# AutonomousVehicleLaboratory/vision_semantic_segmentation

Hardware: AMD Instinct MI355X
Metric: fused frames/sec/GPU (1920x1080 + 120k pts) + max|dlog-odds| vs ref (higher is better)
Workload: dtype f16 hi+lo split, MX-FP4 correction passes, fp32 accumulate

## Files before the change

vision_semantic_segmentation_amd/csrc/seg_gconv_mfma.hip:

```cpp
#include <cstring>

#include "seg_types.h"

namespace avl {
namespace {

constexpr int TW = 32;
constexpr int CC = 64;

template <typename HT>
struct GconvArgs {
    const HT* in;
    const HT* in_lo;
    const HT* w;
    const float* bias;
    HT* out;
    HT* out_lo;
    char* oq[2];
    char* os[2];
    long long o_srows;
    int H, W, in_ld, OH, OW, out_ld, C;
    int stride, dil;
    int th;
    int tiles_x, tiles_y, cchunks;
    int comb;
    int nsp, nslots;
    int walk;
    int tile_bytes;
    int tw_magic;
    const char* w4;
    const char* w4s;
    const char* xq[2];
    const char* xs[2];
    long long x_srows;
    int dephase;
};

template <typename HT, int WS, int NJ, bool XS = false>
__global__ void __launch_bounds__(512) k_gconv_mfma(GconvArgs<HT> p) {
    static_assert(!XS || WS == 1, "a split input goes with split weights");
    typedef typename Half16<HT>::v8 v8;
    extern __shared__ __attribute__((aligned(16))) char lds[];
    const int tid = threadIdx.x, lane = tid & 63;
    const int wave = __builtin_amdgcn_readfirstlane(tid >> 6);
    {
        const long long ipix = (long long)p.H * p.W, opix = (long long)p.OH * p.OW;
        p.in = image_base(p.in, ipix, p.in_ld);
        p.in_lo = image_base(p.in_lo, ipix, p.in_ld);
        p.out = image_base(p.out, opix, p.out_ld);
        p.out_lo = image_base(p.out_lo, opix, p.out_ld);
#pragma unroll
        for (int pl = 0; pl < 2; ++pl) {
            p.oq[pl] = image_base(p.oq[pl], opix, p.C / 2);
            p.os[pl] = image_base(p.os[pl], opix, 8);
            p.xq[pl] = image_base(p.xq[pl], ipix, p.C / 2);
            p.xs[pl] = image_base(p.xs[pl], ipix, 8);
        }
    }
    int bid = blockIdx.x;
    {
        const int nwg = gridDim.x, xcd = bid & 7, local = bid >> 3, q = nwg >> 3, r = nwg & 7;
        bid = (xcd < r ? xcd * (q + 1) : r * (q + 1) + (xcd - r) * q) + local;
    }
    const int cchunk = bid % p.cchunks, slot = bid / p.cchunks;
    const int s = p.stride;
    const int d = p.comb ? 1 : p.dil;
    const int step = p.comb ? p.dil : 1;
    const int in_th = (p.th - 1) * s + 2 * d + 1, in_tw = (TW - 1) * s + 2 * d + 1;
    const int c0 = cchunk * CC;
    const int npix = in_th * in_tw;
    const int ngroups = (npix + 7) >> 3;
    const unsigned lds0 = lds_addr(lds);
    const int n64 = (npix + 63) >> 6;
    const int QBASE = ngroups * 1024, QT = n64 * 1024, SBASE = QBASE + 4 * QT, ST = n64 * 256;
    const bool has_lo = WS == 2 && p.xq[1] != nullptr;
    const int LOBASE = ngroups * 1024;

    const char* const xq0 = p.xq[0];
    const char* const xs0 = p.xs[0];
    const long long xq_delta = has_lo ? p.xq[1] - p.xq[0] : 0, xs_delta = has_lo ? p.xs[1] - p.xs[0] : 0;
    auto stage = [&](int sp, int buf) -> unsigned {
        int tx, ty, cmb;
        if (p.walk) { ty = sp % p.tiles_y; const int r1 = sp / p.tiles_y; tx = r1 % p.tiles_x; cmb = r1 / p.tiles_x; }
        else { tx = sp % p.tiles_x; const int r1 = sp / p.tiles_x; ty = r1 % p.tiles_y; cmb = r1 / p.tiles_y; }
        const int ry = p.comb ? cmb / p.dil : 0, rx = p.comb ? cmb % p.dil : 0;
        const int iy0 = ry + (ty * p.th * s - d) * step, ix0 = rx + (tx * TW * s - d) * step;
        const int prow = lane >> 3, cphys = lane & 7;
        unsigned oob = 0;
        int it = 0;
        for (int gi = wave; gi < ngroups; gi += 8, ++it) {
            const int pix = gi * 8 + prow;
            const int ly = (pix * p.tw_magic) >> 16, lx = pix - ly * in_tw;
            const int iy = iy0 + ly * step, ix = ix0 + lx * step;
            const unsigned outside = (unsigned)(pix >= npix) | (unsigned)((unsigned)iy >= (unsigned)p.H) | (unsigned)((unsigned)ix >= (unsigned)p.W);
            const int cy = min(max(iy, 0), p.H - 1), cx = min(max(ix, 0), p.W - 1);
            const unsigned voff = ((unsigned)(cy * p.W + cx) * (unsigned)p.in_ld + ((cphys ^ (pix & 7)) << 3)) * (unsigned)sizeof(HT);
            glds16_saddr(p.in + c0, voff, lds0 + buf * p.tile_bytes + gi * 1024);
            if constexpr (XS) glds16_saddr(p.in_lo + c0, voff, lds0 + buf * p.tile_bytes + LOBASE + gi * 1024);
            oob |= outside << it;
        }
        if constexpr (WS == 2) {
            const int pwbits = has_lo ? 2 : 1;
            it = 16;
            for (int item = wave; item < (n64 << pwbits); item += 8, ++it) {
                const int pw = item & ((1 << pwbits) - 1), gq = item >> pwbits, w = pw & 1, pl = pw >> 1;
                const int pix = gq * 64 + lane;
                const int ly = (pix * p.tw_magic) >> 16, lx = pix - ly * in_tw;
                const int iy = iy0 + ly * step, ix = ix0 + lx * step;
                const unsigned outside = (unsigned)(pix >= npix) | (unsigned)((unsigned)iy >= (unsigned)p.H) | (unsigned)((unsigned)ix >= (unsigned)p.W);
                const int cy = min(max(iy, 0), p.H - 1), cx = min(max(ix, 0), p.W - 1);
                glds16_saddr(xq0 + pl * xq_delta + c0 / 2 + w * 16, (unsigned)(cy * p.W + cx) * (unsigned)(p.C / 2),
                             lds0 + buf * p.tile_bytes + QBASE + (pl * 2 + w) * QT + gq * 1024);
                oob |= outside << it;
            }
            for (int item = wave; item < (n64 << (pwbits - 1)); item += 8) {
                const int pl = item & ((1 << (pwbits - 1)) - 1), gq = item >> (pwbits - 1);
                const int pix = gq * 64 + lane;
                const int ly = (pix * p.tw_magic) >> 16, lx = pix - ly * in_tw;
                const int cy = min(max(iy0 + ly * step, 0), p.H - 1), cx = min(max(ix0 + lx * step, 0), p.W - 1);
                glds4_saddr(xs0 + pl * xs_delta + ((long long)(c0 >> 8) * p.x_srows) * 8 + ((c0 >> 5) & 4), (unsigned)(cy * p.W + cx) * 8u,
                            lds0 + buf * p.tile_bytes + SBASE + pl * ST + gq * 256);
            }
        }
        return oob;
    };
    const int per = (p.nsp + p.nslots - 1) / p.nslots;
    const int sp_step = p.walk ? 1 : p.nslots, sp_end = p.walk ? min(p.nsp, (slot + 1) * per) : p.nsp;
    int sp = p.walk ? slot * per : slot, buf = 0;
    unsigned oob = sp < sp_end ? stage(sp, 0) : 0u;

    const int win = wave & 1;
    const int part = wave >> 1;
    const int fr = lane & 15, kq = lane >> 4;
    constexpr int NT = WS == 1 ? 18 : 9;
    v8 wf[2][NT];
    {
        const HT* wp = p.w + (long long)(cchunk * 2 + win) * (2 * NT * 16 * 32);
#pragma unroll
        for (int nj = 0; nj < 2; ++nj)
#pragma unroll
            for (int t = 0; t < NT; ++t)
                wf[nj][t] = *reinterpret_cast<const v8*>(wp + ((nj * NT + t) * 16 + fr) * 32 + kq * 8);
    }
    int4 w4[WS == 2 ? 2 : 1][2][3];
    unsigned w4sc[3] = {0u, 0u, 0u};
    if constexpr (WS == 2) {
        const long long widx = cchunk * 2 + win;
        const char* w4p = p.w4 + widx * (2 * 2 * 3 * 64 * 16) + lane * 16;
#pragma unroll
        for (int nj = 0; nj < 2; ++nj)
#pragma unroll
            for (int pr = 0; pr < 2; ++pr)
#pragma unroll
                for (int g = 0; g < 3; ++g) w4[nj][pr][g] = *reinterpret_cast<const int4*>(w4p + ((nj * 2 + pr) * 3 + g) * (64 * 16));
        const unsigned* sp = reinterpret_cast<const unsigned*>(p.w4s + widx * (64 * 12) + lane * 12);
        w4sc[0] = sp[0]; w4sc[1] = sp[1]; w4sc[2] = sp[2];
    }
    const int ssel = 8 * (((c0 >> 5) & 3) + win);
    const int cbase = c0 + win * 32 + kq * 8;
    const int chunk_in = win * 4 + kq;
    f32x4 bias0, bias1;
    {
        const float4 b0 = *reinterpret_cast<const float4*>(p.bias + cbase);
        const float4 b1 = *reinterpret_cast<const float4*>(p.bias + cbase + 4);
        bias0 = f32x4{b0.x, b0.y, b0.z, b0.w};
        bias1 = f32x4{b1.x, b1.y, b1.z, b1.w};
    }

    asm volatile("s_waitcnt vmcnt(0)" ::: "memory");
    auto zero_oob = [&](unsigned mask, int b) {
        if (mask) {
            int it = 0;
            for (int gi = wave; gi < ngroups; gi += 8, ++it)
                if ((mask >> it) & 1u) {
                    *reinterpret_cast<uint4*>(lds + b * p.tile_bytes + gi * 1024 + lane * 16) = make_uint4(0u, 0u, 0u, 0u);
                    if constexpr (XS) *reinterpret_cast<uint4*>(lds + b * p.tile_bytes + LOBASE + gi * 1024 + lane * 16) = make_uint4(0u, 0u, 0u, 0u);
                }
            if constexpr (WS == 2) {
                const int pwbits = has_lo ? 2 : 1;
                it = 16;
                for (int item = wave; item < (n64 << pwbits); item += 8, ++it)
                    if ((mask >> it) & 1u) {
                        const int pw = item & ((1 << pwbits) - 1), gq = item >> pwbits;
                        *reinterpret_cast<uint4*>(lds + b * p.tile_bytes + QBASE + pw * QT + gq * 1024 + lane * 16) = make_uint4(0u, 0u, 0u, 0u);
                    }
            }
        }
    };
    zero_oob(oob, 0);
    __syncthreads();

    constexpr bool HOIST = NJ <= 2 && WS != 2;
    int toff[HOIST ? NJ : 1][9];
    if constexpr (HOIST) {
#pragma unroll
        for (int j = 0; j < NJ; ++j) {
            const int st = part + 4 * j;
            const int sy = st >> 1, sx = (st & 1) * 16 + fr;
#pragma unroll
            for (int t = 0; t < 9; ++t) {
                const int pix = (sy * s + (t / 3) * d) * in_tw + sx * s + (t % 3) * d;
                toff[j][t] = pix * 128 + ((chunk_in ^ (pix & 7)) << 4);
            }
        }
    }
    const unsigned o_ld = (unsigned)p.out_ld, q_ld = (unsigned)(p.C / 2);
    const unsigned sc_lane = (unsigned)(cbase >> 8) * (unsigned)p.o_srows * 8u + (unsigned)((cbase >> 5) & 7);

    for (; sp < sp_end; sp += sp_step, buf ^= 1) {
        const bool late_stage = NJ >= 2 && wave >= 4 && p.dephase;
        oob = 0u;
        if (!late_stage && sp + sp_step < sp_end) oob = stage(sp + sp_step, buf ^ 1);
        const char* tile = lds + buf * p.tile_bytes;
        f32x4 acc[NJ][2];
#pragma unroll
        for (int j = 0; j < NJ; ++j) {
            if (NJ >= 2 && j == NJ / 2 && late_stage && sp + sp_step < sp_end) oob = stage(sp + sp_step, buf ^ 1);
            v8 a[9];
            if constexpr (HOIST) {
#pragma unroll
                for (int t = 0; t < 9; ++t) a[t] = *reinterpret_cast<const v8*>(tile + toff[j][t]);
            } else {
                const int st = part + 4 * j;
                int frv = fr;
                asm volatile("" : "+v"(frv));
                const int sy = st >> 1, sx = (st & 1) * 16 + frv;
#pragma unroll
                for (int t = 0; t < 9; ++t) {
                    const int pix = (sy * s + (t / 3) * d) * in_tw + sx * s + (t % 3) * d;
                    a[t] = *reinterpret_cast<const v8*>(tile + pix * 128 + ((chunk_in ^ (pix & 7)) << 4));
                }
            }
            f32x4 acc0 = bias0, acc1 = bias1;
            if constexpr (WS == 2) {
                typedef int v8i __attribute__((ext_vector_type(8)));
                const int st2 = part + 4 * j;
                const int sy2 = st2 >> 1, sx2 = (st2 & 1) * 16 + fr;
                int4 bq[2][3];
                int bs[2][3];
#pragma unroll
                for (int g = 0; g < 3; ++g) {
                    const int t = min(4 * g + kq, 8);
                    const int pix = (sy2 * s + (t / 3) * d) * in_tw + sx2 * s + (t % 3) * d;
#pragma unroll
                    for (int pl = 0; pl < 2; ++pl) {
                        if (pl == 1 && !has_lo) { bq[pl][g] = make_int4(0, 0, 0, 0); bs[pl][g] = 127; continue; }
                        bq[pl][g] = *reinterpret_cast<const int4*>(tile + QBASE + (pl * 2 + win) * QT + pix * 16);
                        bs[pl][g] = (int)((*reinterpret_cast<const unsigned*>(tile + SBASE + pl * ST + pix * 4) >> ssel) & 0xffu);
                    }
                }
#pragma unroll
                for (int t = 0; t < 9; ++t) {
                    acc0 = Half16<HT>::mfma(wf[0][t], a[t], acc0);
                    acc1 = Half16<HT>::mfma(wf[1][t], a[t], acc1);
                }
#define AVL_GMX(NJ_, PR, G, ACC)                                                                                                \
    {                                                                                                                          \
        const v8i wa = {w4[NJ_][PR][G].x, w4[NJ_][PR][G].y, w4[NJ_][PR][G].z, w4[NJ_][PR][G].w, 0, 0, 0, 0};                    \
        const v8i xa = {bq[PR][G].x, bq[PR][G].y, bq[PR][G].z, bq[PR][G].w, 0, 0, 0, 0};                                        \
        ACC = __builtin_amdgcn_mfma_scale_f32_16x16x128_f8f6f4(wa, xa, ACC, 4, 4, ((NJ_) * 6 + (PR) * 3 + (G)) & 3,              \
                                                               (int)w4sc[((NJ_) * 6 + (PR) * 3 + (G)) >> 2], 0, bs[PR][G]);     \
    }
                AVL_GMX(0, 0, 0, acc0) AVL_GMX(0, 0, 1, acc0) AVL_GMX(0, 0, 2, acc0)
                AVL_GMX(1, 0, 0, acc1) AVL_GMX(1, 0, 1, acc1) AVL_GMX(1, 0, 2, acc1)
                if (has_lo) {
                    AVL_GMX(0, 1, 0, acc0) AVL_GMX(0, 1, 1, acc0) AVL_GMX(0, 1, 2, acc0)
                    AVL_GMX(1, 1, 0, acc1) AVL_GMX(1, 1, 1, acc1) AVL_GMX(1, 1, 2, acc1)
                }
#undef AVL_GMX
            } else {
#pragma unroll
                for (int t = 0; t < 9; ++t) {
                    acc0 = Half16<HT>::mfma(wf[0][t], a[t], acc0);
                    acc1 = Half16<HT>::mfma(wf[1][t], a[t], acc1);
                    if constexpr (WS == 1) {
                        acc0 = Half16<HT>::mfma(wf[0][9 + t], a[t], acc0);
                        acc1 = Half16<HT>::mfma(wf[1][9 + t], a[t], acc1);
                    }
                }
                if constexpr (XS) {
                    if constexpr (HOIST) {
#pragma unroll
                        for (int t = 0; t < 9; ++t) a[t] = *reinterpret_cast<const v8*>(tile + LOBASE + toff[j][t]);
                    } else {
                        const int st = part + 4 * j;
                        int frv = fr;
                        asm volatile("" : "+v"(frv));
                        const int sy = st >> 1, sx = (st & 1) * 16 + frv;
#pragma unroll
                        for (int t = 0; t < 9; ++t) {
                            const int pix = (sy * s + (t / 3) * d) * in_tw + sx * s + (t % 3) * d;
                            a[t] = *reinterpret_cast<const v8*>(tile + LOBASE + pix * 128 + ((chunk_in ^ (pix & 7)) << 4));
                        }
                    }
#pragma unroll
                    for (int t = 0; t < 9; ++t) {
                        acc0 = Half16<HT>::mfma(wf[0][t], a[t], acc0);
                        acc1 = Half16<HT>::mfma(wf[1][t], a[t], acc1);
                    }
                }
            }
            acc[j][0] = acc0; acc[j][1] = acc1;
            __builtin_amdgcn_sched_barrier(0);
        }
        asm volatile("s_waitcnt vmcnt(0)" ::: "memory");
        zero_oob(oob, buf ^ 1);

        int tx, ty, cmb;
        if (p.walk) { ty = sp % p.tiles_y; const int r1 = sp / p.tiles_y; tx = r1 % p.tiles_x; cmb = r1 / p.tiles_x; }
        else { tx = sp % p.tiles_x; const int r1 = sp / p.tiles_x; ty = r1 % p.tiles_y; cmb = r1 / p.tiles_y; }
        const int ry = p.comb ? cmb / p.dil : 0, rx = p.comb ? cmb % p.dil : 0;
        const int oy0 = ty * p.th, ox0 = tx * TW;
#pragma unroll
        for (int j = 0; j < NJ; ++j) {
            const int st = part + 4 * j;
            const int sy = st >> 1, sx = (st & 1) * 16 + fr;
            const int oy = ry + (oy0 + sy) * step, ox = rx + (ox0 + sx) * step;
            const bool live = oy < p.OH && ox < p.OW;
            const unsigned pix = live ? (unsigned)oy * (unsigned)p.OW + (unsigned)ox : 0u;
            float v[8];
#pragma unroll
            for (int r = 0; r < 4; ++r) {
                v[r] = fmaxf(acc[j][0][r], 0.f);
                v[4 + r] = fmaxf(acc[j][1][r], 0.f);
            }
            if constexpr (WS == 0) {
                if (live) Vec8<HT>::store(p.out + (pix * o_ld + (unsigned)cbase), v);
            } else {
                typedef typename Half16<HT>::v8 h8;
                typedef HT h2 __attribute__((ext_vector_type(2)));
                typedef unsigned u4 __attribute__((ext_vector_type(4)));
                u4 hpk;
#pragma unroll
                for (int r = 0; r < 4; ++r) {
                    const h2 t = {(HT)v[2 * r], (HT)v[2 * r + 1]};
                    hpk[r] = __builtin_bit_cast(unsigned, t);
                }
                const h8 hv = __builtin_bit_cast(h8, hpk);
                if (live) *reinterpret_cast<h8*>(p.out + (pix * o_ld + (unsigned)cbase)) = hv;
                float lo[8];
#pragma unroll
                for (int r = 0; r < 8; ++r) {
                    const float h = (float)hv[r];
                    lo[r] = v[r] - h;
                    v[r] = h;
                }
                if (p.out_lo) {
                    h8 lv;
#pragma unroll
                    for (int r = 0; r < 8; ++r) lv[r] = (HT)lo[r];
                    if (live) *reinterpret_cast<h8*>(p.out_lo + (pix * o_ld + (unsigned)cbase)) = lv;
#pragma unroll
                    for (int r = 0; r < 8; ++r) lo[r] = (float)lv[r];
                }
#pragma unroll
                for (int pl = 0; pl < 2; ++pl) {
                    if (p.oq[pl] == nullptr) continue;
                    const float* src = pl == 0 ? v : lo;
                    float amax = 0.f;
#pragma unroll
                    for (int r = 0; r < 8; ++r) amax = fmaxf(amax, fabsf(src[r]));
                    {
                        const unsigned ab = __float_as_uint(amax);
                        const auto r16 = __builtin_amdgcn_permlane16_swap(ab, ab, false, false);
                        const unsigned m16 = max(r16[0], r16[1]);
                        const auto r32 = __builtin_amdgcn_permlane32_swap(m16, m16, false, false);
                        amax = __uint_as_float(max(r32[0], r32[1]));
                    }
                    const unsigned sbyte = mx_fp4_scale_byte(amax);
                    const float scale = __uint_as_float(sbyte << 23);
                    unsigned pk = 0u;
                    pk = __builtin_amdgcn_cvt_scalef32_pk_fp4_f32(pk, src[0], src[1], scale, 0);
                    pk = __builtin_amdgcn_cvt_scalef32_pk_fp4_f32(pk, src[2], src[3], scale, 1);
                    pk = __builtin_amdgcn_cvt_scalef32_pk_fp4_f32(pk, src[4], src[5], scale, 2);
                    pk = __builtin_amdgcn_cvt_scalef32_pk_fp4_f32(pk, src[6], src[7], scale, 3);
                    if (live) {
                        *reinterpret_cast<unsigned*>(p.oq[pl] + (pix * q_ld + (unsigned)(cbase / 2))) = pk;
                        if (kq == 0) p.os[pl][sc_lane + pix * 8u] = (char)sbyte;
                    }
                }
            }
            __builtin_amdgcn_sched_barrier(0);
        }
        __syncthreads();
    }
}

}

int gconv_mfma_lds_bytes(int stride, int dil, int& th) {
    th = stride == 1 ? 8 : 4;
    const int in_th = (th - 1) * stride + 2 * dil + 1, in_tw = (TW - 1) * stride + 2 * dil + 1;
    return ((in_th * in_tw + 7) / 8) * 1024;
}

static int gconv_tile_bytes(int stride, int dil, int th, bool mx = false, bool xs = false) {
    const int in_th = (th - 1) * stride + 2 * dil + 1, in_tw = (TW - 1) * stride + 2 * dil + 1;
    const int npix = in_th * in_tw, n64 = (npix + 63) / 64;
    return ((npix + 7) / 8) * 1024 * (xs ? 2 : 1) + (mx ? 4 * n64 * 1024 + 2 * n64 * 256 : 0);
}

static int device_cus() {
    static int n = 0;
    if (n == 0) {
        int dev = 0;
        hipDeviceProp_t prop;
        if (hipGetDevice(&dev) == hipSuccess && hipGetDeviceProperties(&prop, dev) == hipSuccess) n = prop.multiProcessorCount;
        if (n <= 0) n = 256;
    }
    return n;
}

static int gconv_pick_th(const avl_seg_op& op, int comb, int cus, int* nsp_out, int* nslots_out) {
    const bool mx = op.w_split == 2, xs = op.in_lo != nullptr;
    const int d = comb ? 1 : op.dil;
    const int gh = comb ? (op.out_h + op.dil - 1) / op.dil : op.out_h, gw = comb ? (op.out_w + op.dil - 1) / op.dil : op.out_w;
    const int ncomb = comb ? op.dil * op.dil : 1, cchunks = op.in_c / CC;
    int best = 0;
    double best_cost = 0.;
    for (int th = 8; th >= 2; th >>= 1) {
        if (2 * gconv_tile_bytes(op.stride, d, th, mx, xs) > 160 * 1024) continue;
        if ((mx || xs) && th == 8) continue;
        const int nsp = ((gw + TW - 1) / TW) * ((gh + th - 1) / th) * ncomb;
        int nslots = cus / cchunks;
        if (nslots < 1) nslots = 1;
        if (nslots > nsp) nslots = nsp;
        const int rounds = (nsp + nslots - 1) / nslots;
        const double cost = (double)rounds * (th + 0.5);
        if (th == 2 && best != 0) break;
        if (best == 0 || cost < best_cost) {
            best = th; best_cost = cost;
            *nsp_out = nsp; *nslots_out = nslots;
        }
    }
    return best;
}

template <typename HT, int WS, bool XS = false>
int launch_gconv_typed(const avl_seg_op& op, hipStream_t s) {
    GconvArgs<HT> a;
    a.in = static_cast<const HT*>(op.in);
    a.in_lo = static_cast<const HT*>(op.in_lo);
    a.w = static_cast<const HT*>(op.weight);
    a.bias = op.bias;
    a.out = static_cast<HT*>(op.out);
    a.out_lo = static_cast<HT*>(op.out_lo);
    a.oq[0] = a.oq[1] = a.os[0] = a.os[1] = nullptr;
    a.o_srows = op.out_rows;
    if (op.out_mx) {
        const auto o = mx_bundle(op.out_mx, op.out_rows, op.out_c);
        a.oq[0] = o.q[0]; a.os[0] = o.s[0];
        if (op.out_lo || (op.mx_flags & AVL_MX_OUT_LO)) { a.oq[1] = o.q[1]; a.os[1] = o.s[1]; }
    }
    a.H = op.in_h; a.W = op.in_w; a.in_ld = op.in_ld; a.OH = op.out_h; a.OW = op.out_w; a.out_ld = op.out_ld; a.C = op.in_c;
    a.stride = op.stride; a.dil = op.dil;
    a.comb = (op.stride == 1 && op.dil > 1 && op.pad == op.dil) ? 1 : 0;
    a.th = gconv_pick_th(op, a.comb, device_cus(), &a.nsp, &a.nslots);
    AVL_REQUIRE(a.th > 0, "grouped conv: no tile height fits two LDS buffers");
    a.tile_bytes = gconv_tile_bytes(op.stride, a.comb ? 1 : op.dil, a.th, WS == 2, XS);
    a.w4 = a.w4s = a.xq[0] = a.xq[1] = a.xs[0] = a.xs[1] = nullptr;
    a.x_srows = op.in_rows;
    if (WS == 2) {
        const long long nwin = op.in_c / 32;
        a.w4 = static_cast<const char*>(op.w_mx);
        a.w4s = a.w4 + nwin * (2 * 2 * 3 * 64 * 16);
        const auto x = mx_bundle(op.in_mx, op.in_rows, op.in_c);
        a.xq[0] = x.q[0]; a.xs[0] = x.s[0];
        if (op.mx_flags & AVL_MX_IN_LO) { a.xq[1] = x.q[1]; a.xs[1] = x.s[1]; }
    }
    {
        const int d = a.comb ? 1 : op.dil;
        const int in_th = (a.th - 1) * op.stride + 2 * d + 1, in_tw = (TW - 1) * op.stride + 2 * d + 1;
        a.tw_magic = (65536 + in_tw - 1) / in_tw;
        for (int pix = 0; pix < ((in_th * in_tw + 63) / 64) * 64; ++pix)
            AVL_REQUIRE(((pix * a.tw_magic) >> 16) == pix / in_tw, "grouped conv: tile %d x %d too large for the reciprocal division", in_th, in_tw);
    }
    const int gh = a.comb ? (op.out_h + op.dil - 1) / op.dil : op.out_h, gw = a.comb ? (op.out_w + op.dil - 1) / op.dil : op.out_w;
    a.tiles_x = (gw + TW - 1) / TW;
    a.tiles_y = (gh + a.th - 1) / a.th;
    a.cchunks = op.in_c / CC;
#define AVL_GCONV_LAUNCH(NJ)                                                                                                          \
    do {                                                                                                                              \
        AVL_HIP_CHECK(hipFuncSetAttribute(reinterpret_cast<const void*>(&k_gconv_mfma<HT, WS, NJ, XS>), hipFuncAttributeMaxDynamicSharedMemorySize, 160 * 1024)); \
        hipLaunchKernelGGL((k_gconv_mfma<HT, WS, NJ, XS>), dim3(a.nslots * a.cchunks, 1, op_batch(op)), dim3(512), 2 * a.tile_bytes, s, a); \
    } while (0)
    a.dephase = 1;
    a.walk = 1;
    if (a.th == 8) {
        if constexpr (WS != 2 && !XS) AVL_GCONV_LAUNCH(4);
        else return avl::set_error(AVL_E_ARG, "MX / split-input grouped conv: tile height 8 is not built");
    }
    else if (a.th == 4) AVL_GCONV_LAUNCH(2);
    else AVL_GCONV_LAUNCH(1);
#undef AVL_GCONV_LAUNCH
    AVL_LAUNCH_CHECK();
    return AVL_OK;
}

int launch_gconv_mfma(const avl_seg_op& op, hipStream_t s) {
    if (op.w_split == 2) return launch_gconv_typed<f16, 2>(op, s);
    if (op.w_split && op.in_lo) return launch_gconv_typed<f16, 1, true>(op, s);
    if (op.w_split) return launch_gconv_typed<f16, 1>(op, s);
    return op.dtype == AVL_F16 ? launch_gconv_typed<f16, 0>(op, s) : launch_gconv_typed<bf16, 0>(op, s);
}

int validate_gconv_mfma(const avl_seg_op& op) {
    AVL_REQUIRE(is_half(op.dtype), "MFMA grouped conv needs a 16-bit activation type");
    AVL_REQUIRE(op.in_c % CC == 0, "MFMA grouped conv needs channels %% 64 == 0 (got %d)", op.in_c);
    AVL_REQUIRE(!op.w_split || op.dtype == AVL_F16, "split weights need AVL_F16 activations");
    AVL_REQUIRE(!op.in2_lo && (!op.out_lo || op.w_split) && (!op.in_lo || op.w_split == 1), "grouped conv: a split output needs w_split, a split input w_split = 1");
    AVL_REQUIRE(!op.in_lo || reinterpret_cast<uintptr_t>(op.in_lo) % 16 == 0, "grouped conv: unaligned lo plane");
    if (op.w_split == 2) {
        AVL_REQUIRE(op.w_mx && op.in_mx && op.in_c % 256 == 0 && op.in_ld == op.in_c, "MX grouped conv: w_mx, in_mx, channels %% 256 == 0, dense input rows");
        AVL_REQUIRE((reinterpret_cast<uintptr_t>(op.w_mx) | reinterpret_cast<uintptr_t>(op.in_mx)) % 16 == 0, "MX grouped conv: unaligned bundles");
        AVL_REQUIRE(2 * gconv_tile_bytes(op.stride, (op.stride == 1 && op.pad == op.dil) ? 1 : op.dil, 2, true) <= 160 * 1024, "MX grouped conv: two tile buffers do not fit LDS");
        AVL_REQUIRE((long long)op.in_rows * (op.in_c / 2) < (1LL << 31), "MX grouped conv: FP4 plane beyond 2 GB (32-bit DMA offsets)");
    }
    AVL_REQUIRE(!op.out_mx || (op.w_split >= 1 && op.out_c % 256 == 0 && op.out_ld == op.out_c), "grouped conv: out_mx needs w_split, channels %% 256 == 0 and a dense output");
    AVL_REQUIRE(!(op.mx_flags & AVL_MX_OUT_LO) || (op.out_mx && !op.out_lo), "grouped conv: AVL_MX_OUT_LO needs out_mx and no out_lo");
    AVL_REQUIRE((long long)op.in_rows * op.in_ld * 2 < (1LL << 31), "grouped conv: input plane beyond 2 GB (32-bit DMA offsets)");
    AVL_REQUIRE((long long)op.out_rows * op.out_ld * 2 < (1LL << 31) && (long long)(op.out_c / 256 + 1) * op.out_rows * 8 < (1LL << 31),
                "grouped conv: output planes beyond 2 GB (32-bit epilogue addressing)");
    const int cg = op.in_c / op.groups;
    AVL_REQUIRE(cg <= 32 && 32 % cg == 0, "MFMA grouped conv needs <= 32 channels per group dividing 32 (got %d)", cg);
    AVL_REQUIRE(2 * gconv_tile_bytes(op.stride, (op.stride == 1 && op.pad == op.dil) ? 1 : op.dil, 2, false, op.in_lo != nullptr) <= 160 * 1024, "grouped conv: two tile buffers do not fit LDS (dilation %d)", op.dil);
    return AVL_OK;
}

}
```

Measured before the change: 227.9.

## Cache staging pixel geometry in LDS and cut scalar/vector register pressure in gconv

Precomputes each staging pixel's (ly*step, lx*step) offset once per block into an LDS table, so later tile stages look it up instead of redoing the reciprocal division. Tile coordinates advance incrementally instead of using div/mod per step. Kernel arguments are re-read from the kernarg segment inside the stage and epilogue to shorten SGPR live ranges, and address arithmetic moves to 24-bit multiplies with the batch offset applied per pixel. It costs extra LDS when the table fits and adds range checks that reject large images or batches.

```diff
diff --git a/vision_semantic_segmentation_amd/csrc/seg_gconv_mfma.hip b/vision_semantic_segmentation_amd/csrc/seg_gconv_mfma.hip
--- a/vision_semantic_segmentation_amd/csrc/seg_gconv_mfma.hip
+++ b/vision_semantic_segmentation_amd/csrc/seg_gconv_mfma.hip
@@ -1,4 +1,5 @@
 #include <cstring>
+#include <type_traits>
 
 #include "seg_types.h"
 
@@ -25,7 +26,7 @@
     int tiles_x, tiles_y, cchunks;
     int comb;
     int nsp, nslots;
-    int walk;
+    int geo;
     int tile_bytes;
     int tw_magic;
     const char* w4;
@@ -33,6 +34,7 @@
     const char* xq[2];
     const char* xs[2];
     long long x_srows;
+    long long x_lo;
     int dephase;
 };
 
@@ -43,20 +45,6 @@
     extern __shared__ __attribute__((aligned(16))) char lds[];
     const int tid = threadIdx.x, lane = tid & 63;
     const int wave = __builtin_amdgcn_readfirstlane(tid >> 6);
-    {
-        const long long ipix = (long long)p.H * p.W, opix = (long long)p.OH * p.OW;
-        p.in = image_base(p.in, ipix, p.in_ld);
-        p.in_lo = image_base(p.in_lo, ipix, p.in_ld);
-        p.out = image_base(p.out, opix, p.out_ld);
-        p.out_lo = image_base(p.out_lo, opix, p.out_ld);
-#pragma unroll
-        for (int pl = 0; pl < 2; ++pl) {
-            p.oq[pl] = image_base(p.oq[pl], opix, p.C / 2);
-            p.os[pl] = image_base(p.os[pl], opix, 8);
-            p.xq[pl] = image_base(p.xq[pl], ipix, p.C / 2);
-            p.xs[pl] = image_base(p.xs[pl], ipix, 8);
-        }
-    }
     int bid = blockIdx.x;
     {
         const int nwg = gridDim.x, xcd = bid & 7, local = bid >> 3, q = nwg >> 3, r = nwg & 7;
@@ -72,62 +60,110 @@
     const int ngroups = (npix + 7) >> 3;
     const unsigned lds0 = lds_addr(lds);
     const int n64 = (npix + 63) >> 6;
-    const int QBASE = ngroups * 1024, QT = n64 * 1024, SBASE = QBASE + 4 * QT, ST = n64 * 256;
-    const bool has_lo = WS == 2 && p.xq[1] != nullptr;
+    enum { F_HAS_LO = 1, F_GEO = 2, F_LATE = 4 };
+    unsigned fl = (WS == 2 && p.xq[1] != nullptr ? F_HAS_LO : 0) | (p.geo ? F_GEO : 0) | (NJ >= 2 && wave >= 4 && p.dephase ? F_LATE : 0);
+    fl = __builtin_amdgcn_readfirstlane(fl);
+    asm volatile("" : "+s"(fl));
+    auto has_lo = [&]() -> bool { return WS == 2 && (fl & F_HAS_LO) != 0; };
     const int LOBASE = ngroups * 1024;
 
-    const char* const xq0 = p.xq[0];
-    const char* const xs0 = p.xs[0];
-    const long long xq_delta = has_lo ? p.xq[1] - p.xq[0] : 0, xs_delta = has_lo ? p.xs[1] - p.xs[0] : 0;
-    auto stage = [&](int sp, int buf) -> unsigned {
-        int tx, ty, cmb;
-        if (p.walk) { ty = sp % p.tiles_y; const int r1 = sp / p.tiles_y; tx = r1 % p.tiles_x; cmb = r1 / p.tiles_x; }
-        else { tx = sp % p.tiles_x; const int r1 = sp / p.tiles_x; ty = r1 % p.tiles_y; cmb = r1 / p.tiles_y; }
-        const int ry = p.comb ? cmb / p.dil : 0, rx = p.comb ? cmb % p.dil : 0;
-        const int iy0 = ry + (ty * p.th * s - d) * step, ix0 = rx + (tx * TW * s - d) * step;
+    struct Tile { int ty, tx, ry, rx; };
+    auto advance = [&](Tile t) -> Tile {
+        ++t.ty;
+        if (t.ty >= p.tiles_y) {
+            t.ty = 0; ++t.tx;
+            if (t.tx >= p.tiles_x) {
+                t.tx = 0; ++t.rx;
+                if (t.rx >= p.dil) { t.rx = 0; ++t.ry; }
+            }
+        }
+        return t;
+    };
+    auto geo_table = [&](int tile_bytes) -> unsigned* { return reinterpret_cast<unsigned*>(lds + 2 * tile_bytes); };
+    auto geom = [&](int pix, int magic) -> unsigned {
+        const int ly = (pix * magic) >> 16, lx = pix - ly * in_tw;
+        return pix < npix ? ((unsigned)(ly * step) << 12) | (unsigned)(lx * step) : 1u << 31;
+    };
+    const int c0_ = c0, ngroups_ = ngroups, n64_ = n64, lane_ = lane, wave_ = wave;
+    const unsigned lds0_ = lds0;
+    auto stage = [&](Tile t, int buf, auto first) -> unsigned {
+        auto ka = __builtin_amdgcn_kernarg_segment_ptr();
+        asm volatile("" : "+s"(ka));
+        const GconvArgs<HT> e = *(const GconvArgs<HT>*)ka;
+        int c0 = c0_, ngroups = ngroups_, n64 = n64_, lane = lane_, wave = wave_;
+        unsigned lds0 = lds0_;
+        asm volatile("" : "+s"(c0), "+s"(ngroups), "+s"(n64), "+s"(wave), "+s"(lds0));
+        asm volatile("" : "+v"(lane));
+        const int QBASE = ngroups * 1024, QT = n64 * 1024, SBASE = QBASE + 4 * QT, ST = n64 * 256, LOBASE = ngroups * 1024;
+        const int iy0 = t.ry + (t.ty * e.th * s - d) * step, ix0 = t.rx + (t.tx * TW * s - d) * step;
         const int prow = lane >> 3, cphys = lane & 7;
+        const unsigned img_row = blockIdx.z * (unsigned)(e.H * e.W);
+        const unsigned H = (unsigned)e.H, W = (unsigned)e.W;
+        const unsigned tile0 = lds0 + buf * e.tile_bytes;
+        const unsigned* const geo = geo_table(e.tile_bytes);
         unsigned oob = 0;
-        int it = 0;
-        for (int gi = wave; gi < ngroups; gi += 8, ++it) {
-            const int pix = gi * 8 + prow;
-            const int ly = (pix * p.tw_magic) >> 16, lx = pix - ly * in_tw;
-            const int iy = iy0 + ly * step, ix = ix0 + lx * step;
-            const unsigned outside = (unsigned)(pix >= npix) | (unsigned)((unsigned)iy >= (unsigned)p.H) | (unsigned)((unsigned)ix >= (unsigned)p.W);
-            const int cy = min(max(iy, 0), p.H - 1), cx = min(max(ix, 0), p.W - 1);
-            const unsigned voff = ((unsigned)(cy * p.W + cx) * (unsigned)p.in_ld + ((cphys ^ (pix & 7)) << 3)) * (unsigned)sizeof(HT);
-            glds16_saddr(p.in + c0, voff, lds0 + buf * p.tile_bytes + gi * 1024);
-            if constexpr (XS) glds16_saddr(p.in_lo + c0, voff, lds0 + buf * p.tile_bytes + LOBASE + gi * 1024);
-            oob |= outside << it;
-        }
-        if constexpr (WS == 2) {
-            const int pwbits = has_lo ? 2 : 1;
-            it = 16;
-            for (int item = wave; item < (n64 << pwbits); item += 8, ++it) {
-                const int pw = item & ((1 << pwbits) - 1), gq = item >> pwbits, w = pw & 1, pl = pw >> 1;
-                const int pix = gq * 64 + lane;
-                const int ly = (pix * p.tw_magic) >> 16, lx = pix - ly * in_tw;
-                const int iy = iy0 + ly * step, ix = ix0 + lx * step;
-                const unsigned outside = (unsigned)(pix >= npix) | (unsigned)((unsigned)iy >= (unsigned)p.H) | (unsigned)((unsigned)ix >= (unsigned)p.W);
-                const int cy = min(max(iy, 0), p.H - 1), cx = min(max(ix, 0), p.W - 1);
-                glds16_saddr(xq0 + pl * xq_delta + c0 / 2 + w * 16, (unsigned)(cy * p.W + cx) * (unsigned)(p.C / 2),
-                             lds0 + buf * p.tile_bytes + QBASE + (pl * 2 + w) * QT + gq * 1024);
+        auto items = [&](auto tab) {
+            auto look = [&](int pix) -> unsigned { if constexpr (decltype(tab)::value) return geo[pix]; else return geom(pix, e.tw_magic); };
+            auto row_of = [&](unsigned g, unsigned& outside) -> unsigned {
+                const int iy = iy0 + (int)(g >> 12), ix = ix0 + (int)(g & 0xfffu);
+                outside = (unsigned)((unsigned)iy >= H) | (unsigned)((unsigned)ix >= W);
+                const unsigned cy = (unsigned)min(max(iy, 0), (int)H - 1), cx = (unsigned)min(max(ix, 0), (int)W - 1);
+                return __umul24(cy, W) + cx + img_row;
+            };
+            int it = 0;
+            unsigned g = look(wave * 8 + prow);
+            for (int gi = wave; gi < ngroups; gi += 8, ++it) {
+                const unsigned gn = look((gi + 8) * 8 + prow);
+                unsigned outside;
+                const unsigned voff = (__umul24(row_of(g, outside), (unsigned)e.in_ld) + ((cphys ^ prow) << 3)) * (unsigned)sizeof(HT);
+                glds16_saddr(e.in + c0, voff, tile0 + gi * 1024);
+                if constexpr (XS) glds16_saddr(e.in_lo + c0, voff, tile0 + LOBASE + gi * 1024);
                 oob |= outside << it;
-            }
-            for (int item = wave; item < (n64 << (pwbits - 1)); item += 8) {
-                const int pl = item & ((1 << (pwbits - 1)) - 1), gq = item >> (pwbits - 1);
-                const int pix = gq * 64 + lane;
-                const int ly = (pix * p.tw_magic) >> 16, lx = pix - ly * in_tw;
-                const int cy = min(max(iy0 + ly * step, 0), p.H - 1), cx = min(max(ix0 + lx * step, 0), p.W - 1);
-                glds4_saddr(xs0 + pl * xs_delta + ((long long)(c0 >> 8) * p.x_srows) * 8 + ((c0 >> 5) & 4), (unsigned)(cy * p.W + cx) * 8u,
-                            lds0 + buf * p.tile_bytes + SBASE + pl * ST + gq * 256);
-            }
-        }
+                g = gn;
+            }
+            if constexpr (WS == 2) {
+                const int pwbits = has_lo() ? 2 : 1;
+                const char* const xq0 = e.xq[0] + c0 / 2;
+                const char* const xs0 = e.xs[0] + ((long long)(c0 >> 8) * e.x_srows) * 8 + ((c0 >> 5) & 4);
+                const long long xq_delta = e.x_lo, xs_delta = e.x_lo;
+                const unsigned q_ld = (unsigned)(e.C / 2);
+                it = 16;
+                g = look((wave >> pwbits) * 64 + lane);
+                for (int item = wave; item < (n64 << pwbits); item += 8, ++it) {
+                    const int pw = item & ((1 << pwbits) - 1), gq = item >> pwbits, w = pw & 1, pl = pw >> 1;
+                    const unsigned gn = look(((item + 8) >> pwbits) * 64 + lane);
+                    unsigned outside;
+                    const unsigned voff = __umul24(row_of(g, outside), q_ld);
+                    glds16_saddr(xq0 + pl * xq_delta + w * 16, voff, tile0 + QBASE + (pl * 2 + w) * QT + gq * 1024);
+                    oob |= outside << it;
+                    g = gn;
+                }
+                g = look((wave >> (pwbits - 1)) * 64 + lane);
+                for (int item = wave; item < (n64 << (pwbits - 1)); item += 8) {
+                    const int pl = item & ((1 << (pwbits - 1)) - 1), gq = item >> (pwbits - 1);
+                    const unsigned gn = look(((item + 8) >> (pwbits - 1)) * 64 + lane);
+                    unsigned outside;
+                    glds4_saddr(xs0 + pl * xs_delta, row_of(g, outside) * 8u, tile0 + SBASE + pl * ST + gq * 256);
+                    g = gn;
+                }
+            }
+        };
+        if (!decltype(first)::value && (fl & F_GEO)) items(std::true_type{});
+        else items(std::false_type{});
         return oob;
     };
     const int per = (p.nsp + p.nslots - 1) / p.nslots;
-    const int sp_step = p.walk ? 1 : p.nslots, sp_end = p.walk ? min(p.nsp, (slot + 1) * per) : p.nsp;
-    int sp = p.walk ? slot * per : slot, buf = 0;
-    unsigned oob = sp < sp_end ? stage(sp, 0) : 0u;
+    const int sp_end = min(p.nsp, (slot + 1) * per);
+    int sp = slot * per, buf = 0;
+    Tile cur;
+    {
+        const int ty = sp % p.tiles_y, r1 = sp / p.tiles_y, tx = r1 % p.tiles_x, cmb = r1 / p.tiles_x;
+        cur.ty = ty; cur.tx = tx;
+        cur.ry = p.comb ? cmb / p.dil : 0; cur.rx = p.comb ? cmb % p.dil : 0;
+    }
+    unsigned oob = sp < sp_end ? stage(cur, 0, std::true_type{}) : 0u;
+    if (fl & F_GEO)
+        for (int pix = tid; pix < n64 * 64; pix += 512) geo_table(p.tile_bytes)[pix] = geom(pix, p.tw_magic);
 
     const int win = wave & 1;
     const int part = wave >> 1;
@@ -170,6 +206,9 @@
     asm volatile("s_waitcnt vmcnt(0)" ::: "memory");
     auto zero_oob = [&](unsigned mask, int b) {
         if (mask) {
+            int ng = ngroups, n6 = n64;
+            asm volatile("" : "+s"(ng), "+s"(n6));
+            const int ngroups = ng, n64 = n6, QBASE = ng * 1024, QT = n6 * 1024, LOBASE = ng * 1024;
             int it = 0;
             for (int gi = wave; gi < ngroups; gi += 8, ++it)
                 if ((mask >> it) & 1u) {
@@ -177,7 +216,7 @@
                     if constexpr (XS) *reinterpret_cast<uint4*>(lds + b * p.tile_bytes + LOBASE + gi * 1024 + lane * 16) = make_uint4(0u, 0u, 0u, 0u);
                 }
             if constexpr (WS == 2) {
-                const int pwbits = has_lo ? 2 : 1;
+                const int pwbits = has_lo() ? 2 : 1;
                 it = 16;
                 for (int item = wave; item < (n64 << pwbits); item += 8, ++it)
                     if ((mask >> it) & 1u) {
@@ -204,18 +243,18 @@
             }
         }
     }
-    const unsigned o_ld = (unsigned)p.out_ld, q_ld = (unsigned)(p.C / 2);
     const unsigned sc_lane = (unsigned)(cbase >> 8) * (unsigned)p.o_srows * 8u + (unsigned)((cbase >> 5) & 7);
 
-    for (; sp < sp_end; sp += sp_step, buf ^= 1) {
-        const bool late_stage = NJ >= 2 && wave >= 4 && p.dephase;
+    for (; sp < sp_end; ++sp, buf ^= 1, cur = advance(cur)) {
+        asm volatile("" : "+s"(fl));
+        const bool late_stage = (fl & F_LATE) != 0;
         oob = 0u;
-        if (!late_stage && sp + sp_step < sp_end) oob = stage(sp + sp_step, buf ^ 1);
+        if (!late_stage && sp + 1 < sp_end) oob = stage(advance(cur), buf ^ 1, std::false_type{});
         const char* tile = lds + buf * p.tile_bytes;
         f32x4 acc[NJ][2];
 #pragma unroll
         for (int j = 0; j < NJ; ++j) {
-            if (NJ >= 2 && j == NJ / 2 && late_stage && sp + sp_step < sp_end) oob = stage(sp + sp_step, buf ^ 1);
+            if (NJ >= 2 && j == NJ / 2 && late_stage && sp + 1 < sp_end) oob = stage(advance(cur), buf ^ 1, std::false_type{});
             v8 a[9];
             if constexpr (HOIST) {
 #pragma unroll
@@ -224,16 +263,21 @@
                 const int st = part + 4 * j;
                 int frv = fr;
                 asm volatile("" : "+v"(frv));
+                int sv = s, dv = d, twv = in_tw;
+                asm volatile("" : "+s"(sv), "+s"(dv), "+s"(twv));
                 const int sy = st >> 1, sx = (st & 1) * 16 + frv;
 #pragma unroll
                 for (int t = 0; t < 9; ++t) {
-                    const int pix = (sy * s + (t / 3) * d) * in_tw + sx * s + (t % 3) * d;
+                    const int pix = (sy * sv + (t / 3) * dv) * twv + sx * sv + (t % 3) * dv;
                     a[t] = *reinterpret_cast<const v8*>(tile + pix * 128 + ((chunk_in ^ (pix & 7)) << 4));
                 }
             }
             f32x4 acc0 = bias0, acc1 = bias1;
             if constexpr (WS == 2) {
                 typedef int v8i __attribute__((ext_vector_type(8)));
+                int ng = ngroups, n6 = n64;
+                asm volatile("" : "+s"(ng), "+s"(n6));
+                const int QBASE = ng * 1024, QT = n6 * 1024, SBASE = QBASE + 4 * QT, ST = n6 * 256;
                 const int st2 = part + 4 * j;
                 const int sy2 = st2 >> 1, sx2 = (st2 & 1) * 16 + fr;
                 int4 bq[2][3];
@@ -244,7 +288,7 @@
                     const int pix = (sy2 * s + (t / 3) * d) * in_tw + sx2 * s + (t % 3) * d;
 #pragma unroll
                     for (int pl = 0; pl < 2; ++pl) {
-                        if (pl == 1 && !has_lo) { bq[pl][g] = make_int4(0, 0, 0, 0); bs[pl][g] = 127; continue; }
+                        if (pl == 1 && !has_lo()) { bq[pl][g] = make_int4(0, 0, 0, 0); bs[pl][g] = 127; continue; }
                         bq[pl][g] = *reinterpret_cast<const int4*>(tile + QBASE + (pl * 2 + win) * QT + pix * 16);
                         bs[pl][g] = (int)((*reinterpret_cast<const unsigned*>(tile + SBASE + pl * ST + pix * 4) >> ssel) & 0xffu);
                     }
@@ -263,7 +307,7 @@
     }
                 AVL_GMX(0, 0, 0, acc0) AVL_GMX(0, 0, 1, acc0) AVL_GMX(0, 0, 2, acc0)
                 AVL_GMX(1, 0, 0, acc1) AVL_GMX(1, 0, 1, acc1) AVL_GMX(1, 0, 2, acc1)
-                if (has_lo) {
+                if (has_lo()) {
                     AVL_GMX(0, 1, 0, acc0) AVL_GMX(0, 1, 1, acc0) AVL_GMX(0, 1, 2, acc0)
                     AVL_GMX(1, 1, 0, acc1) AVL_GMX(1, 1, 1, acc1) AVL_GMX(1, 1, 2, acc1)
                 }
@@ -303,21 +347,22 @@
             acc[j][0] = acc0; acc[j][1] = acc1;
             __builtin_amdgcn_sched_barrier(0);
         }
+        auto ka = __builtin_amdgcn_kernarg_segment_ptr();
+        asm volatile("" : "+s"(ka));
+        const GconvArgs<HT> e = *(const GconvArgs<HT>*)ka;
         asm volatile("s_waitcnt vmcnt(0)" ::: "memory");
         zero_oob(oob, buf ^ 1);
 
-        int tx, ty, cmb;
-        if (p.walk) { ty = sp % p.tiles_y; const int r1 = sp / p.tiles_y; tx = r1 % p.tiles_x; cmb = r1 / p.tiles_x; }
-        else { tx = sp % p.tiles_x; const int r1 = sp / p.tiles_x; ty = r1 % p.tiles_y; cmb = r1 / p.tiles_y; }
-        const int ry = p.comb ? cmb / p.dil : 0, rx = p.comb ? cmb % p.dil : 0;
-        const int oy0 = ty * p.th, ox0 = tx * TW;
+        const unsigned o_ld = (unsigned)e.out_ld, q_ld = (unsigned)(e.C / 2);
+        const unsigned img_row = blockIdx.z * (unsigned)(e.OH * e.OW);
+        const int ry = cur.ry, rx = cur.rx, oy0 = cur.ty * e.th, ox0 = cur.tx * TW;
 #pragma unroll
         for (int j = 0; j < NJ; ++j) {
             const int st = part + 4 * j;
             const int sy = st >> 1, sx = (st & 1) * 16 + fr;
             const int oy = ry + (oy0 + sy) * step, ox = rx + (ox0 + sx) * step;
-            const bool live = oy < p.OH && ox < p.OW;
-            const unsigned pix = live ? (unsigned)oy * (unsigned)p.OW + (unsigned)ox : 0u;
+            const bool live = oy < e.OH && ox < e.OW;
+            const unsigned pix = live ? img_row + (unsigned)oy * (unsigned)e.OW + (unsigned)ox : 0u;
             float v[8];
 #pragma unroll
             for (int r = 0; r < 4; ++r) {
@@ -325,7 +370,7 @@
                 v[4 + r] = fmaxf(acc[j][1][r], 0.f);
             }
             if constexpr (WS == 0) {
-                if (live) Vec8<HT>::store(p.out + (pix * o_ld + (unsigned)cbase), v);
+                if (live) Vec8<HT>::store(e.out + (pix * o_ld + (unsigned)cbase), v);
             } else {
                 typedef typename Half16<HT>::v8 h8;
                 typedef HT h2 __attribute__((ext_vector_type(2)));
@@ -337,7 +382,7 @@
                     hpk[r] = __builtin_bit_cast(unsigned, t);
                 }
                 const h8 hv = __builtin_bit_cast(h8, hpk);
-                if (live) *reinterpret_cast<h8*>(p.out + (pix * o_ld + (unsigned)cbase)) = hv;
+                if (live) *reinterpret_cast<h8*>(e.out + (pix * o_ld + (unsigned)cbase)) = hv;
                 float lo[8];
 #pragma unroll
                 for (int r = 0; r < 8; ++r) {
@@ -345,17 +390,17 @@
                     lo[r] = v[r] - h;
                     v[r] = h;
                 }
-                if (p.out_lo) {
+                if (e.out_lo) {
                     h8 lv;
 #pragma unroll
                     for (int r = 0; r < 8; ++r) lv[r] = (HT)lo[r];
-                    if (live) *reinterpret_cast<h8*>(p.out_lo + (pix * o_ld + (unsigned)cbase)) = lv;
+                    if (live) *reinterpret_cast<h8*>(e.out_lo + (pix * o_ld + (unsigned)cbase)) = lv;
 #pragma unroll
                     for (int r = 0; r < 8; ++r) lo[r] = (float)lv[r];
                 }
 #pragma unroll
                 for (int pl = 0; pl < 2; ++pl) {
-                    if (p.oq[pl] == nullptr) continue;
+                    if (e.oq[pl] == nullptr) continue;
                     const float* src = pl == 0 ? v : lo;
                     float amax = 0.f;
 #pragma unroll
@@ -375,8 +420,8 @@
                     pk = __builtin_amdgcn_cvt_scalef32_pk_fp4_f32(pk, src[4], src[5], scale, 2);
                     pk = __builtin_amdgcn_cvt_scalef32_pk_fp4_f32(pk, src[6], src[7], scale, 3);
                     if (live) {
-                        *reinterpret_cast<unsigned*>(p.oq[pl] + (pix * q_ld + (unsigned)(cbase / 2))) = pk;
-                        if (kq == 0) p.os[pl][sc_lane + pix * 8u] = (char)sbyte;
+                        *reinterpret_cast<unsigned*>(e.oq[pl] + (pix * q_ld + (unsigned)(cbase / 2))) = pk;
+                        if (kq == 0) e.os[pl][sc_lane + pix * 8u] = (char)sbyte;
                     }
                 }
             }
@@ -398,6 +443,11 @@
     const int in_th = (th - 1) * stride + 2 * dil + 1, in_tw = (TW - 1) * stride + 2 * dil + 1;
     const int npix = in_th * in_tw, n64 = (npix + 63) / 64;
     return ((npix + 7) / 8) * 1024 * (xs ? 2 : 1) + (mx ? 4 * n64 * 1024 + 2 * n64 * 256 : 0);
+}
+
+static int gconv_geo_bytes(int stride, int dil, int th) {
+    const int in_th = (th - 1) * stride + 2 * dil + 1, in_tw = (TW - 1) * stride + 2 * dil + 1;
+    return ((in_th * in_tw + 63) / 64 + 8) * 64 * 4;
 }
 
 static int device_cus() {
@@ -460,18 +510,27 @@
     a.tile_bytes = gconv_tile_bytes(op.stride, a.comb ? 1 : op.dil, a.th, WS == 2, XS);
     a.w4 = a.w4s = a.xq[0] = a.xq[1] = a.xs[0] = a.xs[1] = nullptr;
     a.x_srows = op.in_rows;
+    a.x_lo = 0;
     if (WS == 2) {
         const long long nwin = op.in_c / 32;
         a.w4 = static_cast<const char*>(op.w_mx);
         a.w4s = a.w4 + nwin * (2 * 2 * 3 * 64 * 16);
         const auto x = mx_bundle(op.in_mx, op.in_rows, op.in_c);
         a.xq[0] = x.q[0]; a.xs[0] = x.s[0];
-        if (op.mx_flags & AVL_MX_IN_LO) { a.xq[1] = x.q[1]; a.xs[1] = x.s[1]; }
+        if (op.mx_flags & AVL_MX_IN_LO) {
+            a.xq[1] = x.q[1]; a.xs[1] = x.s[1];
+            a.x_lo = x.q[1] - x.q[0];
+            AVL_REQUIRE(x.s[1] - x.s[0] == a.x_lo, "MX grouped conv: the halves of the input bundle are laid out differently");
+        }
     }
     {
         const int d = a.comb ? 1 : op.dil;
         const int in_th = (a.th - 1) * op.stride + 2 * d + 1, in_tw = (TW - 1) * op.stride + 2 * d + 1;
         a.tw_magic = (65536 + in_tw - 1) / in_tw;
+        AVL_REQUIRE(in_tw * op.dil < (1 << 12) && in_th * op.dil < (1 << 18) && op.in_h + 2 * op.dil * op.dil < (1 << 18),
+                    "grouped conv: image height %d / dilation %d beyond the staging geometry's range", op.in_h, op.dil);
+        AVL_REQUIRE((long long)op_batch(op) * op.in_h * op.in_w < (1 << 24) && op.in_ld < (1 << 24), "grouped conv: more than 2^24 input pixels or channels (24-bit address arithmetic)");
+        a.geo = 2 * a.tile_bytes + gconv_geo_bytes(op.stride, d, a.th) <= 160 * 1024 ? 1 : 0;
         for (int pix = 0; pix < ((in_th * in_tw + 63) / 64) * 64; ++pix)
             AVL_REQUIRE(((pix * a.tw_magic) >> 16) == pix / in_tw, "grouped conv: tile %d x %d too large for the reciprocal division", in_th, in_tw);
     }
@@ -482,10 +541,9 @@
 #define AVL_GCONV_LAUNCH(NJ)                                                                                                          \
     do {                                                                                                                              \
         AVL_HIP_CHECK(hipFuncSetAttribute(reinterpret_cast<const void*>(&k_gconv_mfma<HT, WS, NJ, XS>), hipFuncAttributeMaxDynamicSharedMemorySize, 160 * 1024)); \
-        hipLaunchKernelGGL((k_gconv_mfma<HT, WS, NJ, XS>), dim3(a.nslots * a.cchunks, 1, op_batch(op)), dim3(512), 2 * a.tile_bytes, s, a); \
+        hipLaunchKernelGGL((k_gconv_mfma<HT, WS, NJ, XS>), dim3(a.nslots * a.cchunks, 1, op_batch(op)), dim3(512), 2 * a.tile_bytes + (a.geo ? gconv_geo_bytes(op.stride, a.comb ? 1 : op.dil, a.th) : 0), s, a); \
     } while (0)
     a.dephase = 1;
-    a.walk = 1;
     if (a.th == 8) {
         if constexpr (WS != 2 && !XS) AVL_GCONV_LAUNCH(4);
         else return avl::set_error(AVL_E_ARG, "MX / split-input grouped conv: tile height 8 is not built");
```

Result: no change. 229.7 (median of 6 runs) (+0.8%).
